# bootphon/shennong

Hardware: AMD Instinct MI355X
Metric: frames/s (25 ms/10 ms, 16 kHz) for fbank-40 + MFCC-13 at 1/2/4/8 GPUs (higher is better)
Workload: dtype f32

## Files before the change

include/shennong_amd.h:

```cpp
#ifndef SHENNONG_AMD_H_
#define SHENNONG_AMD_H_

#include <stdint.h>

#ifdef __cplusplus
extern "C" {
#endif

#define SNF_OK 0
#define SNF_E_INVALID (-1)
#define SNF_E_RUNTIME (-2)
#define SNF_E_HIP (-3)
#define SNF_E_NODEVICE (-4)

#define SNF_KIND_SPECTROGRAM 0
#define SNF_KIND_FBANK 1
#define SNF_KIND_MFCC 2
#define SNF_KIND_PLP 3
#define SNF_KIND_PITCH 4
#define SNF_KIND_PITCH_POST 5
#define SNF_KIND_DELTA 6
#define SNF_KIND_ENERGY 7
#define SNF_KIND_VAD 8
#define SNF_KIND_CMVN 9
// ... 332 lines not shown
int snf_memcpy_h2d_async(void* dst, const void* src, uint64_t bytes, void* stream);
int snf_memcpy_d2h_async(void* dst, const void* src, uint64_t bytes, void* stream);
int snf_event_create(void** event);
int snf_event_destroy(void* event);
int snf_event_record(void* event, void* stream);
int snf_event_synchronize(void* event);
int snf_stream_wait_event(void* stream, void* event);
int snf_event_elapsed_ms(void* start, void* stop, float* ms);
int snf_host_malloc(void** hptr, uint64_t bytes);
int snf_host_free(void* hptr);
int snf_wav_scan(const char* path, int32_t* channels, int32_t* sample_rate, int64_t* nsamples, int32_t* bits,
                 int32_t* format_tag);
int snf_wav_read_pcm16(const char* const* paths, int64_t n_files, const int64_t* first_sample,
                       const int64_t* n_samples, int16_t* dst, const int64_t* dst_offsets, int32_t threads,
                       int32_t* status);

#define SNF_COMM_ID_BYTES 128
typedef struct snf_comm snf_comm;
int snf_comm_unique_id(void* id128);
int snf_comm_init(const void* id128, int32_t world_size, int32_t rank, int32_t device_id, snf_comm** out);
int snf_comm_rank(const snf_comm* comm);
int snf_comm_world_size(const snf_comm* comm);
int snf_comm_destroy(snf_comm* comm);
int snf_comm_gatherv(snf_comm* comm, const float* d_send, int64_t send_count, float* d_recv,
                     const int64_t* recv_counts, int32_t root, void* stream);
int snf_comm_allreduce_f64(snf_comm* comm, double* d_buf, int64_t count, int32_t op, void* stream);

int snf_debug_fill_lds(uint32_t pattern);
int snf_debug_pitch_scratch(snf_plan* plan, void** down, void** nccf_res, void** pov_nccf,
                            void** states);
int snf_debug_plp_tail(snf_plan* plan, const float* mel, const double* energy,
                       const int64_t* frame_offsets, int64_t n_utts, float* out, float* mel_out);
int snf_debug_fbank512b_rel32(const int64_t* sample_offsets, const int64_t* frame_offsets, int64_t n_utts);
float snf_plan_last_kernel_ms(const snf_plan* plan, int which);
const char* snf_plan_kernel_name(const snf_plan* plan, int which);

#ifdef __cplusplus
}
#endif
#endif
```

shennong_amd/_backend.py:

```python

import ctypes as C
import os
import threading

import numpy as np

from shennong_amd import _abi

_HERE = os.path.dirname(os.path.abspath(__file__))
_LIB_PATH = os.environ.get('SHENNONG_AMD_LIB') or os.path.join(_HERE, 'libshennong_hip.so')
_LIB = None
_LOCK = threading.Lock()
_PLANS = {}
_DEVICE = int(os.environ.get('SHENNONG_AMD_DEVICE', '0'))

EXPORTS = [
    'snf_version', 'snf_last_error', 'snf_device_count', 'snf_set_device',
    'snf_device_name', 'snf_device_synchronize', 'snf_num_frames',
    'snf_first_sample_of_frame', 'snf_window_size', 'snf_window_shift',
    'snf_padded_window_size', 'snf_window_function', 'snf_pitch_num_frames',
    'snf_plan_create', 'snf_plan_destroy', 'snf_plan_ndims', 'snf_plan_fast_path',
    'snf_plan_num_frames', 'snf_plan_run_batch', 'snf_plan_run_batch_device',
    'snf_post_ndims', 'snf_post_run_batch', 'snf_post_run_batch_device',
    'snf_cmvn_accumulate', 'snf_cmvn_apply', 'snf_cmvn_accumulate_device',
    'snf_cmvn_apply_device', 'snf_concat_columns_device', 'snf_count_nonfinite_device', 'snf_set_noise_call',
    'snf_malloc', 'snf_free', 'snf_memcpy_h2d', 'snf_memcpy_d2h', 'snf_memset',
    'snf_host_malloc', 'snf_host_free', 'snf_debug_fill_lds', 'snf_debug_pitch_scratch',
    'snf_debug_plp_tail', 'snf_debug_fbank512b_rel32',
    'snf_stream_create', 'snf_stream_destroy', 'snf_stream_synchronize', 'snf_memcpy_h2d_async',
    'snf_memcpy_d2h_async', 'snf_comm_unique_id', 'snf_comm_init', 'snf_comm_rank', 'snf_comm_world_size',
    'snf_comm_destroy', 'snf_comm_gatherv', 'snf_comm_allreduce_f64',
    'snf_plan_last_kernel_ms', 'snf_plan_kernel_name', 'snf_set_oom_hook',
    'snf_event_create', 'snf_event_destroy', 'snf_event_record', 'snf_event_elapsed_ms', 'snf_mem_info',
    'snf_stream_wait_event', 'snf_stream_query', 'snf_event_synchronize', 'snf_wav_scan', 'snf_wav_read_pcm16',
    'snf_gmm_loglikes', 'snf_gmm_accumulate', 'snf_gmm_gselect', 'snf_gmm_gselect_preselect',
    'snf_gmm_selection_posteriors', 'snf_gmm_posteriors', 'snf_fmllr_accumulate', 'snf_vtln_gram', 'snf_lvtln_select',
    'snf_affine_apply_segments', 'snf_vtln_gram_rows', 'snf_dense_layer', 'snf_bottleneck_vad',
    'snf_bottleneck_fbank', 'snf_bottleneck_nn_input', 'snf_bottleneck_forward', 'snf_crepe_conv',
    'snf_crepe_forward', 'snf_crepe_decode', 'snf_framed_onehot', 'snf_packed_weights_bf16_size',
    'snf_pack_weights_bf16', 'snf_dense_layer_bf16', 'snf_bottleneck_forward_bf16', 'snf_crepe_conv_bf16',
    'snf_crepe_forward_bf16', 'snf_resample_num_out', 'snf_linear_resample', 'snf_crepe_rows',
    'snf_crepe_voicing_convert', 'snf_bottleneck_extract', 'snf_bottleneck_extract_runs',
    'snf_collate_num_out', 'snf_collate_padded', 'snf_dtw_pairs', 'snf_dtw_search', 'snf_dtw_detect', 'snf_dtw_topk',
    'snf_dtw_align',
    'snf_abx_cells']


_OOM_HOOK_TYPE = C.CFUNCTYPE(None)


def _release_pool():
    try:
        DEVICE_POOL.clear()
    except Exception:
        pass


_OOM_HOOK = _OOM_HOOK_TYPE(_release_pool)


def lib():
# ... 36 lines not shown
        L.snf_plan_fast_path.argtypes = [vp]
        L.snf_plan_num_frames.argtypes = [vp, i64]
        L.snf_plan_num_frames.restype = i64
        L.snf_plan_run_batch.argtypes = [vp, pi16, pi64, i64, pf, pf, pi64]
        L.snf_plan_run_batch_device.argtypes = [
            vp, vp, pi64, i64, pf, vp, pi64, vp]
        L.snf_post_ndims.argtypes = [vp, i32]
        L.snf_post_run_batch.argtypes = [vp, pf, i32, pi64, i64, pf]
        L.snf_post_run_batch_device.argtypes = [vp, vp, i32, pi64, i64, vp, vp]
        pi32, pf64 = C.POINTER(C.c_int32), C.POINTER(C.c_double)
        L.snf_cmvn_accumulate.argtypes = [
            vp, pf, i32, pi64, i64, pf, pi32, i32, pf64]
        L.snf_cmvn_apply.argtypes = [
            vp, pf, i32, pi64, i64, pf64, pi32, i32, i32, i32, pf]
        L.snf_cmvn_accumulate_device.argtypes = [
            vp, vp, i32, pi64, i64, vp, pi32, i32, pf64]
        L.snf_cmvn_apply_device.argtypes = [
            vp, vp, i32, pi64, i64, pf64, pi32, i32, i32, i32, vp]
        L.snf_concat_columns_device.argtypes = [
            i32, vp, i32, pi64, vp, i32, pi64, i64, vp, pi64]
        L.snf_count_nonfinite_device.argtypes = [i32, vp, C.c_uint64, C.POINTER(C.c_uint64)]
        L.snf_set_noise_call.argtypes = [C.c_uint64]
        L.snf_malloc.argtypes = [C.POINTER(vp), C.c_uint64]
        L.snf_free.argtypes = [vp]
        L.snf_memcpy_h2d.argtypes = [vp, vp, C.c_uint64]
        L.snf_memcpy_d2h.argtypes = [vp, vp, C.c_uint64]
        L.snf_memset.argtypes = [vp, i32, C.c_uint64]
        L.snf_host_malloc.argtypes = [C.POINTER(vp), C.c_uint64]
        L.snf_host_free.argtypes = [vp]
        L.snf_debug_fill_lds.argtypes = [C.c_uint32]
        L.snf_debug_pitch_scratch.argtypes = [vp] + [C.POINTER(vp)] * 4
        L.snf_debug_plp_tail.argtypes = [vp, pf, C.POINTER(C.c_double), pi64, i64, pf, pf]
        L.snf_debug_fbank512b_rel32.argtypes = [pi64, pi64, i64]
        L.snf_stream_create.argtypes = [C.POINTER(vp)]
        L.snf_stream_destroy.argtypes = [vp]
        L.snf_stream_synchronize.argtypes = [vp]
        L.snf_stream_query.argtypes = [vp]
        L.snf_memcpy_h2d_async.argtypes = [vp, vp, C.c_uint64, vp]
        L.snf_event_create.argtypes = [C.POINTER(vp)]
        L.snf_event_destroy.argtypes = [vp]
        L.snf_event_record.argtypes = [vp, vp]
        L.snf_stream_wait_event.argtypes = [vp, vp]
        L.snf_event_synchronize.argtypes = [vp]
        L.snf_event_elapsed_ms.argtypes = [vp, vp, C.POINTER(C.c_float)]
        L.snf_memcpy_d2h_async.argtypes = [vp, vp, C.c_uint64, vp]
        L.snf_comm_unique_id.argtypes = [vp]
        L.snf_comm_init.argtypes = [vp, i32, i32, i32, C.POINTER(vp)]
        L.snf_comm_rank.argtypes = [vp]
        L.snf_comm_world_size.argtypes = [vp]
        L.snf_comm_destroy.argtypes = [vp]
        L.snf_comm_gatherv.argtypes = [vp, vp, i64, vp, pi64, i32, vp]
        L.snf_comm_allreduce_f64.argtypes = [vp, vp, i64, i32, vp]
        L.snf_plan_last_kernel_ms.argtypes = [vp, i32]
        L.snf_plan_last_kernel_ms.restype = f32
        L.snf_plan_kernel_name.argtypes = [vp, i32]
        L.snf_plan_kernel_name.restype = C.c_char_p
        L.snf_set_oom_hook.argtypes = [_OOM_HOOK_TYPE]
        L.snf_mem_info.argtypes = [C.POINTER(C.c_uint64), C.POINTER(C.c_uint64)]
        L.snf_wav_scan.argtypes = [C.c_char_p, pi32, pi32, pi64, pi32, pi32]
        L.snf_wav_read_pcm16.argtypes = [C.POINTER(C.c_char_p), i64, pi64, pi64, pi16, pi64, i32, pi32]
        L.snf_gmm_loglikes.argtypes = [i32, vp, i64, i32, vp, vp, vp, i32, vp, vp]
        L.snf_gmm_accumulate.argtypes = [i32, vp, i64, i32, vp, vp, vp, vp, i32, vp, vp, vp, vp]
        L.snf_gmm_gselect.argtypes = [i32, vp, i64, i32, vp, vp, vp, i32, i32, vp, vp, vp]
        L.snf_gmm_gselect_preselect.argtypes = [i32, vp, i64, i32, vp, vp, vp, i32, vp, i32, i32, vp, vp, vp]
        L.snf_gmm_selection_posteriors.argtypes = [i32, vp, i64, i32, vp, vp, vp, i32, vp, i32, f32, vp, vp, vp]
        L.snf_gmm_posteriors.argtypes = [i32, vp, i64, i32, vp, vp, vp, i32, vp, vp, vp]
# ... 1377 lines not shown
```

shennong_amd/csrc/capi_mel.hip:

```cpp
#include "plan.h"

using namespace snf;

namespace {

constexpr float kPairSplitRatio = 8.0f;

int check_offsets(const snf_plan* plan, const int64_t* sample_offsets, const int64_t* frame_offsets,
                  int64_t n_utts) {
  if (sample_offsets[0] != 0 || frame_offsets[0] != 0)
    return set_error(SNF_E_INVALID, "offsets tables must start at 0");
  for (int64_t u = 0; u < n_utts; ++u) {
    const int64_t n = sample_offsets[u + 1] - sample_offsets[u];
    const int64_t f = frame_offsets[u + 1] - frame_offsets[u];
    if (n < 0 || f < 0) return set_error(SNF_E_INVALID, "offsets tables must be non-decreasing");
    if (f != snf_plan_num_frames(plan, n))
      return set_error(SNF_E_INVALID, "frame_offsets do not match snf_plan_num_frames for utterance " +
                                          std::to_string(u));
  }
  return SNF_OK;
}

int run_pitch_device(snf_plan* plan, const int16_t* d_wave, const int64_t* sample_offsets,
                     int64_t n_utts, float* d_out, const int64_t* frame_offsets, hipStream_t s) {
// ... 446 lines not shown
  const size_t nb = static_cast<size_t>(plan->o.mel.num_bins), nc = static_cast<size_t>(plan->ndims);
  DevBuf d_mel, d_energy, d_foff, d_out;
  if ((rc = d_mel.ensure(sizeof(float) * nf * nb))) return rc;
  if ((rc = d_energy.ensure(sizeof(double) * nf))) return rc;
  if ((rc = d_out.ensure(sizeof(float) * nf * nc))) return rc;
  if ((rc = d_foff.upload(std::vector<int64_t>(frame_offsets, frame_offsets + n_utts + 1), s))) return rc;
  SNF_HIP_CHECK(hipMemcpyAsync(d_mel.p, mel, sizeof(float) * nf * nb, hipMemcpyHostToDevice, s));
  SNF_HIP_CHECK(hipMemcpyAsync(d_energy.p, energy, sizeof(double) * nf, hipMemcpyHostToDevice, s));
  BatchArgs b{};
  b.frame_offsets = d_foff.as<int64_t>();
  b.n_utts = n_utts;
  b.total_frames = total_frames;
  begin_timing(plan);
  if (plan->o.rasta) {
    if ((rc = launch_rasta(d_mel.as<float>(), b, static_cast<int>(nb), s))) return rc;
    mark_kernel(plan, "rasta_kernel");
  }
  const char* launched = nullptr;
  rc = launch_plp_tail(plan->pp, b, d_mel.as<float>(), d_energy.as<double>(), d_out.as<float>(), s, &launched);
  if (!rc && launched) mark_kernel(plan, launched);
  if (!rc) {
    SNF_HIP_CHECK(hipMemcpyAsync(out, d_out.p, sizeof(float) * nf * nc, hipMemcpyDeviceToHost, s));
    if (mel_out) SNF_HIP_CHECK(hipMemcpyAsync(mel_out, d_mel.p, sizeof(float) * nf * nb, hipMemcpyDeviceToHost, s));
  }
  SNF_HIP_CHECK(hipStreamSynchronize(s));
  return rc;
}

int snf_debug_fbank512b_rel32(const int64_t* sample_offsets, const int64_t* frame_offsets, int64_t n_utts) {
  if (!sample_offsets || !frame_offsets || n_utts < 0) return set_error(SNF_E_INVALID, "null offsets table");
  return fbank512b_rel32_ok(sample_offsets, frame_offsets, n_utts) ? 1 : 0;
}

}
```

shennong_amd/csrc/kernels_fbank512b.hip:

```cpp
#include <float.h>

#include <cstdlib>
#include <type_traits>

#include "snf_internal.h"
#include "device_fft.h"

namespace snf {

namespace {

typedef unsigned u32x4 __attribute__((ext_vector_type(4)));
typedef unsigned u32x2 __attribute__((ext_vector_type(2)));

constexpr int kWaves = kFast512MaxWaves;
constexpr int kHeaderFloats = kFast512HeaderFloats;
constexpr int kTileRow = kFast512TileRow;
constexpr int kTileBytes = kFast512TileBytes;


}

template <int NJ, int KIND, int ENERGY, bool BST, bool DITHER, int MMQ, int LV, bool REL>
__global__ __launch_bounds__(kWaves * 64, 4) void fbank512b_kernel(const Fast512Params p, const BatchArgs b,
                                                                  float* __restrict__ out,
                                                                  double* __restrict__ energy_out) {
  extern __shared__ __attribute__((aligned(16))) char smem[];
  float* tab = reinterpret_cast<float*>(smem);
  for (int i = threadIdx.x; i < p.table_floats; i += kWaves * 64) tab[i] = p.tables[i];
  __syncthreads();
  const float2* __restrict__ t_win = reinterpret_cast<const float2*>(tab + kHeaderFloats);
  const float2* __restrict__ t_tw16 = t_win + 16 * 18;
  const float2* __restrict__ t_tw512 = t_tw16 + 16 * 18;
  const float4* __restrict__ t_mm_a = reinterpret_cast<const float4*>(tab + p.off_mm_a);
  const float* __restrict__ t_lifter = tab + p.off_lifter;
  const float4* __restrict__ t_dd_v = reinterpret_cast<const float4*>(tab + p.off_dd_v);

  const int lane = threadIdx.x & 63, wid = __builtin_amdgcn_readfirstlane(threadIdx.x >> 6);
  const int l = lane & 15, q = lane >> 4;
  const int tab_bytes = (p.table_floats * 4 + 255) & ~255;
  char* wave_base = smem + tab_bytes + (wid * 4 + q) * kTileBytes;
  float2* tile = reinterpret_cast<float2*>(wave_base);
  float* ptile = reinterpret_cast<float*>(wave_base) + q * 16;
  tile[l * kTileRow + 16] = make_float2(0.0f, 0.0f);
  const int mj = lane & 3;
  const float* __restrict__ mm_lane = tab + p.off_mm_lane + lane;
  const float* __restrict__ mtile =
      reinterpret_cast<const float*>(smem + tab_bytes + (wid * 4 + mj) * kTileBytes) + mj * 16;
  int mm_start_once = 0, mm_out_once = 0;
  if (NJ == 13) {
    mm_start_once = reinterpret_cast<const int*>(mm_lane)[0];
    mm_out_once = reinterpret_cast<const int*>(mm_lane)[64];
  }
  static_assert(MMQ == 0 || (NJ == 13 && (MMQ == 6 || MMQ == 7) && (LV == 3 || LV == 4)), "plans of launch_plan");
  const float4* __restrict__ mm_b_once = reinterpret_cast<const float4*>(mtile + mm_start_once);
  float lifter_once = 1.0f;
  if (NJ == 13 && KIND == SNF_KIND_MFCC) lifter_once = t_lifter[l];

  const float win_len_f = static_cast<float>(p.win_len), inv_win_len = 1.0f / win_len_f;
  using idx_t = typename std::conditional<REL, int, int64_t>::type;
  const idx_t total_frames = static_cast<idx_t>(b.total_frames);
  const idx_t n_sets = (total_frames + 3) >> 2;
  const idx_t set_stride = static_cast<idx_t>(gridDim.x) * kWaves;
  const idx_t last_frame = total_frames - 1;
  idx_t set = static_cast<idx_t>(blockIdx.x) * kWaves + wid;
  if (set >= n_sets) return;

  const bool in_last = 2 * (l + 16 * (NJ - 1)) < p.win_len;
  auto in_window = [&](int j) -> bool {
    if (NJ == 13) return j < NJ - 1 || in_last;
    return 2 * (l + 16 * j) < p.win_len;
  };
  static_assert(!REL || NJ == 13, "set-relative addressing: the 25 ms forms");
  const unsigned q8 = static_cast<unsigned>(q) * 8u;
  auto set_rows_of = [&](const void* table, idx_t s) -> uint64_t {
    int rows = static_cast<int>(total_frames) - static_cast<int>(s) * 4;
    rows = rows < 0 ? 0 : rows;
    asm volatile("" : "+s"(rows));
    rows = rows > 4 ? 4 : rows;
    const __amdgpu_buffer_rsrc_t rsrc = __builtin_amdgcn_make_buffer_rsrc(
        const_cast<char*>(static_cast<const char*>(table)) + static_cast<int64_t>(s) * 32, 0, rows * 8, 0x00020000);
    const u32x2 v = __builtin_amdgcn_raw_buffer_load_b64(rsrc, q8, 0, 0);
    return (static_cast<uint64_t>(v.y) << 32) | v.x;
  };
  auto start_of = [&](idx_t s) -> int64_t {
    if (REL) return static_cast<int64_t>(set_rows_of(b.frame_start, s));
    const int64_t gi = s * 4 + q;
    return b.frame_start[gi < last_frame ? gi : last_frame];
  };
  auto noise_of = [&](idx_t s) -> unsigned long long {
    if (!DITHER) return 0ull;
    if (REL) return set_rows_of(b.frame_noise, s);
    const int64_t gi = s * 4 + q;
    return b.frame_noise[gi < last_frame ? gi : last_frame];
  };
  typedef int __attribute__((aligned(2))) int_a2;
  int raw[NJ];
  const unsigned l4 = 4u * l, off12 = in_last ? l4 + 64u * 12u : 0u;
  auto request = [&](int64_t st) {
    if (REL) {
      const unsigned lo = static_cast<unsigned>(st), hi = static_cast<unsigned>(static_cast<uint64_t>(st) >> 32);
      const unsigned lo0 = __builtin_amdgcn_readfirstlane(lo), hi0 = __builtin_amdgcn_readfirstlane(hi);
      const int64_t st0 = static_cast<int64_t>((static_cast<uint64_t>(hi0) << 32) | lo0);
      const int64_t left = b.rel32_samples - st0;
      unsigned over = static_cast<unsigned>(static_cast<uint64_t>(left) >> 31);
      asm volatile("" : "+s"(over));
      const __amdgpu_buffer_rsrc_t wrsrc = __builtin_amdgcn_make_buffer_rsrc(
          const_cast<int16_t*>(b.wave + st0), 0, over != 0u ? -1 : static_cast<int>(static_cast<unsigned>(left) << 1),
          0x00020000);
      unsigned off = ((lo - lo0) << 1) + l4, last = ((lo - lo0) << 1) + off12;
      asm volatile("" : "+v"(off), "+v"(last));
#pragma unroll
      for (int j = 0; j < NJ - 1; ++j)
        raw[j] = static_cast<int>(__builtin_amdgcn_raw_buffer_load_b32(wrsrc, off + 64u * j, 0, 0));
      raw[NJ - 1] = static_cast<int>(__builtin_amdgcn_raw_buffer_load_b32(wrsrc, last, 0, 0));
      return;
    }
    const int16_t* __restrict__ wp = b.wave + st;
    const int16_t* __restrict__ wl = wp + 2 * l;
#pragma unroll
    for (int j = 0; j < NJ; ++j)
      raw[j] = *reinterpret_cast<const int_a2*>((NJ == 13 && j < NJ - 1) || in_window(j) ? wl + 32 * j : wp);
  };
  float4 w512q[4];
  read_quads<4>(t_tw512 + l * 10, w512q);
  int64_t start_next = start_of(set + set_stride);
  unsigned long long noise_cur = noise_of(set), noise_next = noise_of(set + set_stride);
  request(start_of(set));
  if (BST) {
    const __amdgpu_buffer_rsrc_t none = __builtin_amdgcn_make_buffer_rsrc(out, 0, 0, 0x00020000);
    if (KIND == SNF_KIND_MFCC) __builtin_amdgcn_raw_buffer_store_b32(0u, none, -1, 0, 0);
    else __builtin_amdgcn_raw_buffer_store_b128(u32x4{0u, 0u, 0u, 0u}, none, -1, 0, 2);
  }

  for (; set < n_sets; set += set_stride) {
    const idx_t g = set * 4 + q;
    const bool valid = g <= last_frame;

    float xe[NJ], xo[NJ];
    int part_i = 0;
    float part = 0.0f;
    unsigned dkey_lo = 0, dkey_hi = 0;
    if (DITHER) {
      const unsigned long long k = noise_cur ^ p.seed;
      dkey_lo = fmix32(static_cast<unsigned>(k));
      dkey_hi = fmix32(static_cast<unsigned>(k >> 32) ^ dkey_lo);
      asm volatile("" : "+v"(dkey_lo), "+v"(dkey_hi));
    }
    const float dscale = DITHER ? dither_scale(p.dither) : 0.0f;
#pragma unroll
    for (int j = 0; j < NJ; ++j) {
      xe[j] = static_cast<float>(static_cast<short>(raw[j] & 0xffff));
      xo[j] = static_cast<float>(raw[j] >> 16);
      if (DITHER) {
        add_dither_pair(dkey_lo, dkey_hi, static_cast<unsigned>(l + 16 * j), dscale, xe[j], xo[j]);
        const float s2 = xe[j] + xo[j];
        part += in_window(j) ? s2 : 0.0f;
      } else {
        const int both = __builtin_amdgcn_sdot2(__builtin_bit_cast(short2v, raw[j]), short2v{1, 1}, part_i, false);
        part_i = in_window(j) ? both : part_i;
      }
    }
    if (!DITHER) part = static_cast<float>(part_i);
#pragma unroll
    for (int j = 0; j < NJ; ++j) asm volatile("" : "+v"(xe[j]), "+v"(xo[j]) : : "memory");
    asm volatile("" : "+v"(part) : : "memory");
    request(start_next);
    start_next = start_of(set + 2 * set_stride);
    if (DITHER) {
      noise_cur = noise_next;
      noise_next = noise_of(set + 2 * set_stride);
    }

    float neg_mean = 0.0f;
    if (p.remove_dc) {
      const float sum = row_sum16(part);
      const float qv = sum * inv_win_len;
      neg_mean = -__builtin_fmaf(__builtin_fmaf(-qv, win_len_f, sum), inv_win_len, qv);
      if (DITHER) neg_mean = -sum / win_len_f;
    }
    float2 z[16];
    float e_raw = 0.0f, e_post = 0.0f;
    float rot_prev = xe[0] + neg_mean;
    float left[13];
    if (NJ == 13) {
#pragma unroll
      for (int j = 0; j < 13; ++j) left[j] = dpp_row_ror<0x121>(xo[j] + neg_mean);
      row_head_carry13(left, rot_prev, 0x0001000100010001ull);
    }
#pragma unroll
    for (int jj = 0; jj < 16; jj += 2) {
      float4 w4;
      if (jj < NJ)
        w4 = *reinterpret_cast<const float4*>(__builtin_assume_aligned(t_win + l * 18 + jj, 16));
#pragma unroll
      for (int j = jj; j < jj + 2; ++j) {
        if (j < NJ) {
          const float ae = xe[j] + neg_mean, ao = xo[j] + neg_mean;
          float ap;
          if (NJ == 13) {
            ap = left[j < 13 ? j : 0];
          } else {
            const float rot = dpp_row_ror<0x121>(ao);
            ap = l == 0 ? rot_prev : rot;
            rot_prev = rot;
          }
          const float2 w = (j & 1) ? make_float2(w4.z, w4.w) : make_float2(w4.x, w4.y);
          if (ENERGY == 1 && in_window(j)) e_raw += ae * ae + ao * ao;
          const float ye = (ae - p.preemph * ap) * w.x;
          const float yo = (ao - p.preemph * ae) * w.y;
          z[j] = make_float2(ye, yo);
          if (ENERGY == 2) e_post += ye * ye + yo * yo;
        } else {
          z[j] = make_float2(0.0f, 0.0f);
        }
      }
    }
    float e_lin = 0.0f;
    if (ENERGY != 0) e_lin = row_sum16(ENERGY == 1 ? e_raw : e_post);
    __builtin_amdgcn_sched_barrier(0);

    fft16_lf(z);
#pragma unroll
    for (int k2 = 0; k2 < 16; ++k2) tile[k2 * kTileRow + l] = z[k2];
    wave_lds_order();
    float2 ct[16];
    {
      float4 tw4[8];
      read_tw8_row16(t_tw16 + l * 18, tile + l * kTileRow, tw4, z);
#pragma unroll
      for (int m = 0; m < 16; m += 2) {
        ct[m] = make_float2(tw4[m >> 1].x, tw4[m >> 1].y);
        ct[m + 1] = make_float2(tw4[m >> 1].z, tw4[m >> 1].w);
      }
    }
    __builtin_amdgcn_sched_barrier(0);
    fft16_twin(z, ct);
    __builtin_amdgcn_sched_barrier(0);
    wave_lds_order();

#pragma unroll
    for (int r = 0; r < 8; ++r) tile[r * 16 + l] = z[r + 8];
    wave_lds_order();
    float pk[8], pm[8];
    {
      float2 zpart[8];
      read8_b64_rev128(tile + (16 - l), zpart);
#pragma unroll
      for (int i = 0; i < 4; ++i)
        asm volatile("" : "+v"(w512q[i].x), "+v"(w512q[i].y), "+v"(w512q[i].z), "+v"(w512q[i].w));
#pragma unroll
      for (int k1 = 0; k1 < 8; ++k1) {
        const float2 zk = z[k1];
        const float2 zp = zpart[k1];
        const float2 w = (k1 & 1) ? make_float2(w512q[k1 >> 1].z, w512q[k1 >> 1].w)
                                  : make_float2(w512q[k1 >> 1].x, w512q[k1 >> 1].y);
        const float c_re = zk.x + zp.x, c_im = zk.y - zp.y;
        const float d_re = zk.y + zp.y, d_im = zp.x - zk.x;
        const float u_re = __builtin_fmaf(-w.y, d_im, d_re), u_im = __builtin_fmaf(w.y, d_re, d_im);
        const float a_re = __builtin_fmaf(w.x, u_re, c_re), a_im = __builtin_fmaf(w.x, u_im, c_im);
        const float b_re = __builtin_fmaf(-w.x, u_re, c_re), b_im = __builtin_fmaf(w.x, u_im, -c_im);
        pk[k1] = a_re * a_re + a_im * a_im;
        pm[k1] = b_re * b_re + b_im * b_im;
      }
    }
    if (l == 0) {
      const float dc = z[0].x + z[0].y;
      pk[0] = 4.0f * dc * dc;
// ... 187 lines not shown
            v += w[g4].x * x[g4].x;
            v += w[g4].y * x[g4].y;
            v += w[g4].z * x[g4].z;
            v += w[g4].w * x[g4].w;
          }
        } else {
          write_log_mel();
#pragma unroll 2
          for (int g4 = 0; g4 < p.dd_groups; ++g4) {
            const float4 w = dw[g4 * 16], x = dx[g4];
            v += w.x * x.x;
            v += w.y * x.y;
            v += w.z * x.z;
            v += w.w * x.w;
          }
        }
        v *= NJ == 13 ? lifter_once : t_lifter[l];
        if (l == 0 && p.use_energy) v = log_energy;
        int oc = l;
        if (p.htk_compat) {
          oc = l == 0 ? p.num_ceps - 1 : l - 1;
          if (l == 0 && !p.use_energy)
            v = static_cast<float>(static_cast<double>(v) * 1.4142135623730950488016887);
        }
        if (BST) {
          __builtin_amdgcn_raw_buffer_store_b32(__builtin_bit_cast(unsigned, v), orsrc,
                                                l < p.num_ceps ? (q * p.out_cols + oc) * 4 : -1, 0, 0);
        } else if (valid && l < p.num_ceps) {
          row[oc] = v;
        }
      }
    }
    wave_lds_order();
  }
}

bool fbank512b_shape_ok(const Fast512Params& p, bool per_utt) {
  if (const char* knob = getenv("SNF_FBANK512_OLD"))
    if (knob[0] == '1') return false;
  if (p.dual || p.fused_delta || per_utt) return false;
  if (!p.snip_edges || p.dct_mfma) return false;
  if (p.kind != SNF_KIND_FBANK && p.kind != SNF_KIND_MFCC && p.kind != SNF_KIND_PLP) return false;
  return fast512_lds_bytes(p.table_floats, kWaves, false) <= kFast512LdsBytes;
}
bool fbank512b_rel32_spans_ok(const int64_t* sample_offsets, const int64_t* frame_offsets, int64_t n_utts) {
  constexpr int64_t kLimit = int64_t{1} << 30;
  if (frame_offsets[n_utts] >= kLimit) return false;
  int64_t first[3];
  int held = 0;
  for (int64_t u = 0; u < n_utts; ++u) {
    if (frame_offsets[u + 1] == frame_offsets[u]) continue;
    if (held == 3) {
      if (sample_offsets[u] - first[0] >= kLimit) return false;
      first[0] = first[1];
      first[1] = first[2];
      --held;
    }
    first[held++] = sample_offsets[u];
  }
  return held == 0 || sample_offsets[n_utts] - first[0] < kLimit;
}
bool fbank512b_addr64_knob() {
  const char* knob = getenv("SNF_FBANK512B_ADDR64");
  return knob && knob[0] == '1';
}
bool fbank512b_rel32_ok(const int64_t* sample_offsets, const int64_t* frame_offsets, int64_t n_utts) {
  return !fbank512b_addr64_knob() && fbank512b_rel32_spans_ok(sample_offsets, frame_offsets, n_utts);
}
bool fbank512b_eligible(const Fast512Params& p, const BatchArgs& b) {
  if (p.dither != 0.0f && b.frame_noise == nullptr) return false;
  return fbank512b_shape_ok(p, b.blk_utt != nullptr);
}

namespace {

template <int NJ, int KIND, int ENERGY, bool BST, bool DITHER, int MMQ, int LV, bool REL>
int launch_form(const Fast512Params& q, const BatchArgs& b, float* out, double* energy_out, hipStream_t stream) {
  const size_t lds = fast512_lds_bytes(q.table_floats, kWaves, false);
  const int64_t n_sets = (b.total_frames + 3) / 4;
  int64_t blocks = (n_sets + kWaves - 1) / kWaves;
  if (blocks > 256) blocks = 256;
  auto kern = fbank512b_kernel<NJ, KIND, ENERGY, BST, DITHER, MMQ, LV, REL>;
  if (lds > 64 * 1024)
    SNF_HIP_CHECK(hipFuncSetAttribute(reinterpret_cast<const void*>(kern),
                                      hipFuncAttributeMaxDynamicSharedMemorySize, static_cast<int>(lds)));
  hipLaunchKernelGGL(kern, dim3(static_cast<unsigned>(blocks)), dim3(kWaves * 64), lds, stream, q, b, out,
                     energy_out);
  SNF_HIP_CHECK(hipGetLastError());
  return SNF_OK;
}

template <int NJ, int KIND, int ENERGY, bool BST, bool DITHER, int MMQ, int LV>
int launch_dither(const Fast512Params& q, const BatchArgs& b, float* out, double* energy_out, hipStream_t stream) {
  if constexpr (NJ == 13 && !(KIND == SNF_KIND_MFCC && DITHER && MMQ == 7 && LV == 3)) {
    if (b.rel32_samples > 0)
      return launch_form<NJ, KIND, ENERGY, BST, DITHER, MMQ, LV, true>(q, b, out, energy_out, stream);
  }
  return launch_form<NJ, KIND, ENERGY, BST, DITHER, MMQ, LV, false>(q, b, out, energy_out, stream);
}

template <int NJ, int KIND, int ENERGY, bool BST, bool DITHER>
int launch_plan(const Fast512Params& q, const BatchArgs& b, float* out, double* energy_out, hipStream_t stream) {
  if constexpr (NJ == 13 && (BST || !DITHER)) {
    constexpr bool kFits74 = !(KIND == SNF_KIND_MFCC && DITHER && ENERGY != 0);
    if (q.mm_quads == 7 && q.mm_levels == 4) {
      if constexpr (kFits74)
        return launch_dither<NJ, KIND, ENERGY, BST, DITHER, 7, 4>(q, b, out, energy_out, stream);
      else
        return launch_dither<NJ, KIND, ENERGY, BST, DITHER, 0, 0>(q, b, out, energy_out, stream);
    }
    if (q.mm_quads == 7 && q.mm_levels >= 2)
      return launch_dither<NJ, KIND, ENERGY, BST, DITHER, 7, 3>(q, b, out, energy_out, stream);
    if (q.mm_quads == 6 && q.mm_levels == 4)
      return launch_dither<NJ, KIND, ENERGY, BST, DITHER, 6, 4>(q, b, out, energy_out, stream);
  }
  return launch_dither<NJ, KIND, ENERGY, BST, DITHER, 0, 0>(q, b, out, energy_out, stream);
}

template <int NJ, int KIND, int ENERGY, bool BST>
int launch_one(const Fast512Params& q, const BatchArgs& b, float* out, double* energy_out, hipStream_t stream) {
  if (q.dither != 0.0f) return launch_plan<NJ, KIND, ENERGY, BST, true>(q, b, out, energy_out, stream);
  return launch_plan<NJ, KIND, ENERGY, BST, false>(q, b, out, energy_out, stream);
}

template <int NJ, int KIND>
int launch_energy(const Fast512Params& q, const BatchArgs& b, float* out, double* energy_out, hipStream_t stream) {
  const int energy = q.need_raw ? 1 : (q.need_post ? 2 : 0);
  constexpr bool kCanBst = KIND == SNF_KIND_FBANK || KIND == SNF_KIND_MFCC;
  const bool bst = KIND == SNF_KIND_MFCC || (KIND == SNF_KIND_FBANK && q.num_bins % 4 == 0 && !q.use_energy);
  if (energy == 0) {
    if (kCanBst && bst) return launch_one<NJ, KIND, 0, kCanBst>(q, b, out, energy_out, stream);
// ... 41 lines not shown
    h ^= v;
    h = ((h << 13) | (h >> 19)) * 5u + 0xE6546B64u;
  }
  words[u] = fmix32(h);
}
}

int launch_build_utt_noise(const BatchArgs& b, uint32_t* d_words, hipStream_t stream) {
  if (b.n_utts <= 0) return SNF_OK;
  hipLaunchKernelGGL(build_utt_noise_kernel, dim3(static_cast<unsigned>((b.n_utts + 255) / 256)), dim3(256), 0,
                     stream, b, d_words);
  SNF_HIP_CHECK(hipGetLastError());
  return SNF_OK;
}

int launch_build_frame_noise(const BatchArgs& b, uint64_t* d_keys, hipStream_t stream) {
  if (b.total_frames <= 0) return SNF_OK;
  hipLaunchKernelGGL(build_frame_noise_kernel, dim3(static_cast<unsigned>((b.total_frames + 255) / 256)), dim3(256),
                     0, stream, b, d_keys);
  SNF_HIP_CHECK(hipGetLastError());
  return SNF_OK;
}

int launch_fbank512b(const Fast512Params& p, const BatchArgs& b, float* out, int out_cols, double* energy_out,
                     hipStream_t stream) {
  if (b.total_frames <= 0) return SNF_OK;
  Fast512Params q = p;
  q.out_cols = out_cols;
  if ((p.win_len + 31) / 32 == 13) return launch_kind<13>(q, b, out, energy_out, stream);
  return launch_kind<16>(q, b, out, energy_out, stream);
}

}
```

shennong_amd/csrc/snf_internal.h:

```cpp
#ifndef SNF_INTERNAL_H_
#define SNF_INTERNAL_H_

#include <hip/hip_runtime.h>
#include <stdint.h>

#include <map>
#include <mutex>
#include <string>
#include <vector>

#include "../../include/shennong_amd.h"

namespace snf {

int set_error(int code, const std::string& msg);
const char* last_error();

#define SNF_HIP_CHECK(expr)                                                                  \
  do {                                                                                       \
    hipError_t _e = (expr);                                                                  \
    if (_e != hipSuccess)                                                                    \
      return snf::set_error(SNF_E_HIP, std::string(#expr) + ": " + hipGetErrorString(_e));   \
  } while (0)

// ... 181 lines not shown
  int fused_delta;
  const float* delta_scales;
  int table_floats;
  int table_stride;
  const float* tables;
  int off_mm_a, off_mm_lane, off_dd_a, off_lifter, off_dd_v;
};

bool fast512_eligible(const MelParams& mp, bool any_warp);
bool fast512_dual_eligible(const MelParams& mp);
int fast512_build(const MelParams& mp, const std::vector<float>& window, const MelBanksHost& mb,
                  const std::vector<float>& dct, const std::vector<float>& lifter, bool dual,
                  std::vector<float>* blob, Fast512Params* out);
int launch_build_pair_table(const int64_t* d_frame_offsets, const int64_t* d_sample_offsets,
                            const int64_t* d_pair_offsets, int64_t n_utts, int64_t n_pairs, int win_shift,
                            int win_len, int snip_edges, PairRec* d_pairs, hipStream_t stream);
int launch_build_frame_start(const int64_t* d_frame_offsets, const int64_t* d_sample_offsets,
                             int64_t n_utts, int64_t total_frames, int64_t total_samples, int win_shift,
                             int win_len, int snip_edges, int64_t* d_frame_start, int32_t* d_frame_edge,
                             int32_t* d_frame_utt, hipStream_t stream);
int launch_fbank512(const Fast512Params& p, const BatchArgs& b, float* out, int out_cols,
                    double* energy_out, hipStream_t stream, const char** launched = nullptr);
int launch_fbank256x2(const Fast512Params& p, const BatchArgs& b, float* out, int out_cols,
                      double* energy_out, hipStream_t stream);
int launch_build_frame_noise(const BatchArgs& b, uint64_t* d_keys, hipStream_t stream);
int launch_build_utt_noise(const BatchArgs& b, uint32_t* d_words, hipStream_t stream);
bool fbank512b_eligible(const Fast512Params& p, const BatchArgs& b);
bool fbank512b_shape_ok(const Fast512Params& p, bool per_utt);
bool fbank512b_rel32_spans_ok(const int64_t* sample_offsets, const int64_t* frame_offsets, int64_t n_utts);
bool fbank512b_addr64_knob();
bool fbank512b_rel32_ok(const int64_t* sample_offsets, const int64_t* frame_offsets, int64_t n_utts);
int launch_fbank512b(const Fast512Params& p, const BatchArgs& b, float* out, int out_cols,
                     double* energy_out, hipStream_t stream);

bool fbank2048_eligible(const MelParams& mp);
void fbank2048_tables(const MelParams& mp, const std::vector<float>& window, std::vector<float>* blob);
int launch_fbank2048(const MelParams& p, const BatchArgs& b, const float* tables, float* out, int out_cols,
                     double* energy_out, hipStream_t stream);

bool fbank1024x2_eligible(const MelParams& mp);
void fbank1024x2_tables(const MelParams& mp, const std::vector<float>& window, std::vector<float>* blob);
int launch_fbank1024x2(const MelParams& p, const BatchArgs& b, const float* tables, float* out, int out_cols,
                       double* energy_out, hipStream_t stream);

int launch_mfcc_dct(const float* in, int in_cols, int num_bins, int num_ceps, const float* dct_t, const float* lifter,
                    int use_energy, int htk_compat, int64_t total_frames, float* out, int out_cols,
                    hipStream_t stream);

struct PitchDevTables {
  int first_lag, last_lag, num_lags, num_states, win_size, win_shift, full_len;
  int ar_max_taps, rs_in_unit, rs_out_unit, rs_max_taps;
  int snip_edges, recompute_frame;
  float soft_min_f0, inter_frame_factor, nccf_ballast;
  const float* lags;
  const int* ar_first;
  const int* ar_n;
  const float* ar_w;
  int ar_groups, ar_quad_taps;
  const float* ar_quad_w;
  const int* ar_quad_base;
  const int* rs_first;
  const int* rs_ntaps;
  const float* rs_w;
};
struct PitchBatch {
  const int16_t* wave;
// ... 270 lines not shown
```

Before: 3.484 billion.

## Split fbank512b frame sets into contiguous per-workgroup shares with LDS ticket dealing

Replaces the grid-stride assignment of 4-frame sets to waves with a contiguous balanced share per workgroup. Inside each share, waves draw their next set from an LDS atomic ticket counter, so fast waves take more sets. The lookahead prefetch of sample starts and noise now follows the drawn tickets. This is meant to even out tail imbalance across waves and workgroups, at the cost of extra LDS atomics, readfirstlane waits, and a slightly larger LDS footprint. It also adds an env knob to force the old fixed path, a debug share query, and optional timestamp instrumentation.

```diff
diff --git a/include/shennong_amd.h b/include/shennong_amd.h
--- a/include/shennong_amd.h
+++ b/include/shennong_amd.h
@@ -388,6 +388,7 @@
 int snf_debug_plp_tail(snf_plan* plan, const float* mel, const double* energy,
                        const int64_t* frame_offsets, int64_t n_utts, float* out, float* mel_out);
 int snf_debug_fbank512b_rel32(const int64_t* sample_offsets, const int64_t* frame_offsets, int64_t n_utts);
+int snf_debug_fbank512b_share(int64_t n_sets, int64_t blocks, int64_t block, int64_t* lo, int64_t* hi);
 float snf_plan_last_kernel_ms(const snf_plan* plan, int which);
 const char* snf_plan_kernel_name(const snf_plan* plan, int which);
 
diff --git a/shennong_amd/_backend.py b/shennong_amd/_backend.py
--- a/shennong_amd/_backend.py
+++ b/shennong_amd/_backend.py
@@ -26,7 +26,7 @@
     'snf_cmvn_apply_device', 'snf_concat_columns_device', 'snf_count_nonfinite_device', 'snf_set_noise_call',
     'snf_malloc', 'snf_free', 'snf_memcpy_h2d', 'snf_memcpy_d2h', 'snf_memset',
     'snf_host_malloc', 'snf_host_free', 'snf_debug_fill_lds', 'snf_debug_pitch_scratch',
-    'snf_debug_plp_tail', 'snf_debug_fbank512b_rel32',
+    'snf_debug_plp_tail', 'snf_debug_fbank512b_rel32', 'snf_debug_fbank512b_share',
     'snf_stream_create', 'snf_stream_destroy', 'snf_stream_synchronize', 'snf_memcpy_h2d_async',
     'snf_memcpy_d2h_async', 'snf_comm_unique_id', 'snf_comm_init', 'snf_comm_rank', 'snf_comm_world_size',
     'snf_comm_destroy', 'snf_comm_gatherv', 'snf_comm_allreduce_f64',
@@ -129,6 +129,7 @@
         L.snf_debug_pitch_scratch.argtypes = [vp] + [C.POINTER(vp)] * 4
         L.snf_debug_plp_tail.argtypes = [vp, pf, C.POINTER(C.c_double), pi64, i64, pf, pf]
         L.snf_debug_fbank512b_rel32.argtypes = [pi64, pi64, i64]
+        L.snf_debug_fbank512b_share.argtypes = [i64, i64, i64, pi64, pi64]
         L.snf_stream_create.argtypes = [C.POINTER(vp)]
         L.snf_stream_destroy.argtypes = [vp]
         L.snf_stream_synchronize.argtypes = [vp]
diff --git a/shennong_amd/csrc/capi_mel.hip b/shennong_amd/csrc/capi_mel.hip
--- a/shennong_amd/csrc/capi_mel.hip
+++ b/shennong_amd/csrc/capi_mel.hip
@@ -502,4 +502,11 @@
   return fbank512b_rel32_ok(sample_offsets, frame_offsets, n_utts) ? 1 : 0;
 }
 
-}
+int snf_debug_fbank512b_share(int64_t n_sets, int64_t blocks, int64_t block, int64_t* lo, int64_t* hi) {
+  if (!lo || !hi) return set_error(SNF_E_INVALID, "null output");
+  if (n_sets < 0 || blocks < 0 || block < 0 || block > blocks) return set_error(SNF_E_INVALID, "no such workgroup");
+  fbank512b_share(n_sets, blocks, block, lo, hi);
+  return static_cast<int>(fbank512b_blocks(n_sets));
+}
+
+}
diff --git a/shennong_amd/csrc/kernels_fbank512b.hip b/shennong_amd/csrc/kernels_fbank512b.hip
--- a/shennong_amd/csrc/kernels_fbank512b.hip
+++ b/shennong_amd/csrc/kernels_fbank512b.hip
@@ -21,13 +21,25 @@
 
 }
 
-template <int NJ, int KIND, int ENERGY, bool BST, bool DITHER, int MMQ, int LV, bool REL>
+#ifdef SNF_FBANK512B_STAMPS
+#define SNF_STAMP_PARAM , unsigned long long* __restrict__ stamps
+#define SNF_STAMP_ARG , g_stamps
+constexpr int kStampWords = 8;
+unsigned long long* g_stamps = nullptr;
+#else
+#define SNF_STAMP_PARAM
+#define SNF_STAMP_ARG
+#endif
+template <int NJ, int KIND, int ENERGY, bool BST, bool DITHER, int MMQ, int LV, bool REL, bool DEAL>
 __global__ __launch_bounds__(kWaves * 64, 4) void fbank512b_kernel(const Fast512Params p, const BatchArgs b,
                                                                   float* __restrict__ out,
-                                                                  double* __restrict__ energy_out) {
+                                                                  double* __restrict__ energy_out,
+                                                                  const Fast512bShares shares SNF_STAMP_PARAM) {
   extern __shared__ __attribute__((aligned(16))) char smem[];
   float* tab = reinterpret_cast<float*>(smem);
   for (int i = threadIdx.x; i < p.table_floats; i += kWaves * 64) tab[i] = p.tables[i];
+  unsigned* const ticket = reinterpret_cast<unsigned*>(tab + p.table_floats);
+  if (DEAL && threadIdx.x == 0) *ticket = kWaves;
   __syncthreads();
   const float2* __restrict__ t_win = reinterpret_cast<const float2*>(tab + kHeaderFloats);
   const float2* __restrict__ t_tw16 = t_win + 16 * 18;
@@ -38,7 +50,7 @@
 
   const int lane = threadIdx.x & 63, wid = __builtin_amdgcn_readfirstlane(threadIdx.x >> 6);
   const int l = lane & 15, q = lane >> 4;
-  const int tab_bytes = (p.table_floats * 4 + 255) & ~255;
+  const int tab_bytes = ((p.table_floats + (DEAL ? 1 : 0)) * 4 + 255) & ~255;
   char* wave_base = smem + tab_bytes + (wid * 4 + q) * kTileBytes;
   float2* tile = reinterpret_cast<float2*>(wave_base);
   float* ptile = reinterpret_cast<float*>(wave_base) + q * 16;
@@ -63,8 +75,26 @@
   const idx_t n_sets = (total_frames + 3) >> 2;
   const idx_t set_stride = static_cast<idx_t>(gridDim.x) * kWaves;
   const idx_t last_frame = total_frames - 1;
-  idx_t set = static_cast<idx_t>(blockIdx.x) * kWaves + wid;
-  if (set >= n_sets) return;
+  const idx_t set_lo = DEAL ? static_cast<idx_t>(fbank512b_share_lo(shares, blockIdx.x)) : 0;
+  const idx_t set_end = DEAL ? static_cast<idx_t>(fbank512b_share_lo(shares, blockIdx.x + 1)) : n_sets;
+  idx_t set = DEAL ? set_lo + wid : static_cast<idx_t>(blockIdx.x) * kWaves + wid;
+  if (set >= set_end) return;
+  const idx_t frames_end = DEAL && set_end * 4 < total_frames ? set_end * 4 : total_frames;
+  const unsigned ticket_addr = lds_addr(ticket), ticket_one = 1u;
+  auto draw = [&]() -> unsigned {
+    unsigned t;
+    unsigned long long keep;
+    asm volatile("s_mov_b64 %1, exec\n\ts_mov_b64 exec, 1\n\tds_add_rtn_u32 %0, %2, %3\n\ts_mov_b64 exec, %1"
+                 : "=&v"(t), "=&s"(keep)
+                 : "v"(ticket_addr), "v"(ticket_one)
+                 : "memory");
+    return t;
+  };
+  auto set_of = [&](unsigned t) -> idx_t {
+    unsigned s;
+    asm volatile("s_waitcnt lgkmcnt(0)\n\tv_readfirstlane_b32 %0, %1" : "=s"(s) : "v"(t) : "memory");
+    return set_lo + static_cast<idx_t>(s);
+  };
 
   const bool in_last = 2 * (l + 16 * (NJ - 1)) < p.win_len;
   auto in_window = [&](int j) -> bool {
@@ -74,7 +104,7 @@
   static_assert(!REL || NJ == 13, "set-relative addressing: the 25 ms forms");
   const unsigned q8 = static_cast<unsigned>(q) * 8u;
   auto set_rows_of = [&](const void* table, idx_t s) -> uint64_t {
-    int rows = static_cast<int>(total_frames) - static_cast<int>(s) * 4;
+    int rows = static_cast<int>(frames_end) - static_cast<int>(s) * 4;
     rows = rows < 0 ? 0 : rows;
     asm volatile("" : "+s"(rows));
     rows = rows > 4 ? 4 : rows;
@@ -124,16 +154,30 @@
   };
   float4 w512q[4];
   read_quads<4>(t_tw512 + l * 10, w512q);
-  int64_t start_next = start_of(set + set_stride);
-  unsigned long long noise_cur = noise_of(set), noise_next = noise_of(set + set_stride);
+  idx_t set_n1 = 0, set_n2 = 0;
+  if (DEAL) {
+    const unsigned t1 = draw(), t2 = draw();
+    set_n1 = set_of(t1);
+    set_n2 = set_of(t2);
+  }
+  auto ahead1 = [&]() -> idx_t { return DEAL ? set_n1 : set + set_stride; };
+  auto ahead2 = [&]() -> idx_t { return DEAL ? set_n2 : set + 2 * set_stride; };
+  int64_t start_next = start_of(ahead1());
+  unsigned long long noise_cur = noise_of(set), noise_next = noise_of(ahead1());
   request(start_of(set));
   if (BST) {
     const __amdgpu_buffer_rsrc_t none = __builtin_amdgcn_make_buffer_rsrc(out, 0, 0, 0x00020000);
     if (KIND == SNF_KIND_MFCC) __builtin_amdgcn_raw_buffer_store_b32(0u, none, -1, 0, 0);
     else __builtin_amdgcn_raw_buffer_store_b128(u32x4{0u, 0u, 0u, 0u}, none, -1, 0, 2);
   }
-
-  for (; set < n_sets; set += set_stride) {
+#ifdef SNF_FBANK512B_STAMPS
+  unsigned long long stamp_in, stamp_in_real;
+  unsigned stamp_sets = 0;
+  asm volatile("s_memtime %0\n\ts_memrealtime %1\n\ts_waitcnt lgkmcnt(0)" : "=s"(stamp_in), "=s"(stamp_in_real)
+               : : "memory");
+#endif
+
+  while (set < set_end) {
     const idx_t g = set * 4 + q;
     const bool valid = g <= last_frame;
 
@@ -166,10 +210,10 @@
     for (int j = 0; j < NJ; ++j) asm volatile("" : "+v"(xe[j]), "+v"(xo[j]) : : "memory");
     asm volatile("" : "+v"(part) : : "memory");
     request(start_next);
-    start_next = start_of(set + 2 * set_stride);
+    start_next = start_of(ahead2());
     if (DITHER) {
       noise_cur = noise_next;
-      noise_next = noise_of(set + 2 * set_stride);
+      noise_next = noise_of(ahead2());
     }
 
     float neg_mean = 0.0f;
@@ -221,6 +265,8 @@
     __builtin_amdgcn_sched_barrier(0);
 
     fft16_lf(z);
+    unsigned ticket_n3 = 0;
+    if (DEAL) ticket_n3 = draw();
 #pragma unroll
     for (int k2 = 0; k2 < 16; ++k2) tile[k2 * kTileRow + l] = z[k2];
     wave_lds_order();
@@ -234,6 +280,8 @@
         ct[m + 1] = make_float2(tw4[m >> 1].z, tw4[m >> 1].w);
       }
     }
+    idx_t set_n3 = 0;
+    if (DEAL) set_n3 = set_of(ticket_n3);
     __builtin_amdgcn_sched_barrier(0);
     fft16_twin(z, ct);
     __builtin_amdgcn_sched_barrier(0);
@@ -487,7 +535,35 @@
       }
     }
     wave_lds_order();
-  }
+    if (DEAL) {
+      set = set_n1;
+      set_n1 = set_n2;
+      set_n2 = set_n3;
+    } else {
+      set += set_stride;
+    }
+#ifdef SNF_FBANK512B_STAMPS
+    ++stamp_sets;
+#endif
+  }
+#ifdef SNF_FBANK512B_STAMPS
+  {
+    unsigned long long stamp_out, stamp_out_real;
+    asm volatile("s_memtime %0\n\ts_memrealtime %1\n\ts_waitcnt lgkmcnt(0)" : "=s"(stamp_out), "=s"(stamp_out_real)
+                 : : "memory");
+    if (stamps != nullptr && lane == 0) {
+      unsigned long long* mine = stamps + (static_cast<size_t>(blockIdx.x) * kWaves + wid) * kStampWords;
+      mine[0] = (static_cast<unsigned long long>(blockIdx.x) << 8) | static_cast<unsigned>(wid) | (1ull << 63);
+      mine[1] = __builtin_amdgcn_s_getreg(20 | (31 << 11));
+      mine[2] = __builtin_amdgcn_s_getreg(4 | (31 << 11));
+      mine[3] = stamp_sets;
+      mine[4] = stamp_in;
+      mine[5] = stamp_out;
+      mine[6] = stamp_in_real;
+      mine[7] = stamp_out_real;
+    }
+  }
+#endif
 }
 
 bool fbank512b_shape_ok(const Fast512Params& p, bool per_utt) {
@@ -527,31 +603,54 @@
   return fbank512b_shape_ok(p, b.blk_utt != nullptr);
 }
 
+int64_t fbank512b_blocks(int64_t n_sets) {
+  const int64_t blocks = (n_sets + kWaves - 1) / kWaves;
+  return blocks > 256 ? 256 : blocks;
+}
+void fbank512b_share(int64_t n_sets, int64_t blocks, int64_t b, int64_t* lo, int64_t* hi) {
+  const Fast512bShares s = fbank512b_shares(n_sets, blocks);
+  *lo = fbank512b_share_lo(s, b);
+  *hi = fbank512b_share_lo(s, b + 1);
+}
+static bool fbank512b_fixed_knob() {
+  const char* knob = getenv("SNF_FBANK512B_FIXED");
+  return knob && knob[0] == '1';
+}
+
 namespace {
 
-template <int NJ, int KIND, int ENERGY, bool BST, bool DITHER, int MMQ, int LV, bool REL>
+template <int NJ, int KIND, int ENERGY, bool BST, bool DITHER, int MMQ, int LV, bool REL, bool DEAL>
 int launch_form(const Fast512Params& q, const BatchArgs& b, float* out, double* energy_out, hipStream_t stream) {
-  const size_t lds = fast512_lds_bytes(q.table_floats, kWaves, false);
+  const size_t lds = fast512_lds_bytes(q.table_floats + (DEAL ? 1 : 0), kWaves, false);
   const int64_t n_sets = (b.total_frames + 3) / 4;
-  int64_t blocks = (n_sets + kWaves - 1) / kWaves;
-  if (blocks > 256) blocks = 256;
-  auto kern = fbank512b_kernel<NJ, KIND, ENERGY, BST, DITHER, MMQ, LV, REL>;
+  const int64_t blocks = fbank512b_blocks(n_sets);
+  auto kern = fbank512b_kernel<NJ, KIND, ENERGY, BST, DITHER, MMQ, LV, REL, DEAL>;
   if (lds > 64 * 1024)
     SNF_HIP_CHECK(hipFuncSetAttribute(reinterpret_cast<const void*>(kern),
                                       hipFuncAttributeMaxDynamicSharedMemorySize, static_cast<int>(lds)));
   hipLaunchKernelGGL(kern, dim3(static_cast<unsigned>(blocks)), dim3(kWaves * 64), lds, stream, q, b, out,
-                     energy_out);
+                     energy_out, fbank512b_shares(n_sets, blocks) SNF_STAMP_ARG);
   SNF_HIP_CHECK(hipGetLastError());
   return SNF_OK;
+}
+
+template <int NJ, int KIND, int ENERGY, bool BST, bool DITHER, int MMQ, int LV, bool REL>
+int launch_deal(const Fast512Params& q, const BatchArgs& b, float* out, double* energy_out, hipStream_t stream) {
+  constexpr bool kDealFits = NJ == 13 && !(KIND == SNF_KIND_MFCC && (!BST || (DITHER && MMQ == 7)));
+  if constexpr (kDealFits) {
+    if (!fbank512b_fixed_knob() && fast512_lds_bytes(q.table_floats + 1, kWaves, false) <= kFast512LdsBytes)
+      return launch_form<NJ, KIND, ENERGY, BST, DITHER, MMQ, LV, REL, true>(q, b, out, energy_out, stream);
+  }
+  return launch_form<NJ, KIND, ENERGY, BST, DITHER, MMQ, LV, REL, false>(q, b, out, energy_out, stream);
 }
 
 template <int NJ, int KIND, int ENERGY, bool BST, bool DITHER, int MMQ, int LV>
 int launch_dither(const Fast512Params& q, const BatchArgs& b, float* out, double* energy_out, hipStream_t stream) {
   if constexpr (NJ == 13 && !(KIND == SNF_KIND_MFCC && DITHER && MMQ == 7 && LV == 3)) {
     if (b.rel32_samples > 0)
-      return launch_form<NJ, KIND, ENERGY, BST, DITHER, MMQ, LV, true>(q, b, out, energy_out, stream);
-  }
-  return launch_form<NJ, KIND, ENERGY, BST, DITHER, MMQ, LV, false>(q, b, out, energy_out, stream);
+      return launch_deal<NJ, KIND, ENERGY, BST, DITHER, MMQ, LV, true>(q, b, out, energy_out, stream);
+  }
+  return launch_deal<NJ, KIND, ENERGY, BST, DITHER, MMQ, LV, false>(q, b, out, energy_out, stream);
 }
 
 template <int NJ, int KIND, int ENERGY, bool BST, bool DITHER>
@@ -659,3 +758,9 @@
 }
 
 }
+
+#ifdef SNF_FBANK512B_STAMPS
+extern "C" __attribute__((visibility("default"))) void snf_debug_fbank512b_stamps(void* device_buffer) {
+  snf::g_stamps = static_cast<unsigned long long*>(device_buffer);
+}
+#endif
diff --git a/shennong_amd/csrc/snf_internal.h b/shennong_amd/csrc/snf_internal.h
--- a/shennong_amd/csrc/snf_internal.h
+++ b/shennong_amd/csrc/snf_internal.h
@@ -237,6 +237,21 @@
 bool fbank512b_rel32_ok(const int64_t* sample_offsets, const int64_t* frame_offsets, int64_t n_utts);
 int launch_fbank512b(const Fast512Params& p, const BatchArgs& b, float* out, int out_cols,
                      double* energy_out, hipStream_t stream);
+struct Fast512bShares {
+  int64_t base;
+  int64_t rem;
+};
+inline Fast512bShares fbank512b_shares(int64_t n_sets, int64_t blocks) {
+  return blocks > 0 ? Fast512bShares{n_sets / blocks, n_sets % blocks} : Fast512bShares{0, 0};
+}
+#if defined(__HIPCC__)
+__host__ __device__
+#endif
+inline int64_t fbank512b_share_lo(const Fast512bShares& s, int64_t b) {
+  return b * s.base + (b < s.rem ? b : s.rem);
+}
+void fbank512b_share(int64_t n_sets, int64_t blocks, int64_t b, int64_t* lo, int64_t* hi);
+int64_t fbank512b_blocks(int64_t n_sets);
 
 bool fbank2048_eligible(const MelParams& mp);
 void fbank2048_tables(const MelParams& mp, const std::vector<float>& window, std::vector<float>* blob);
```

Result: faster. 3.749 billion, median of 6 (+7.6%).
